# jpe17/TwoTowerMLRetrieval

Hardware: AMD Instinct MI355X
Metric: queries/sec top-k over 10M x 256-d docs (higher is better)
Workload: dtype f32 results (bit-identical to the fp32 FMA chain); f16-MFMA screen + fp32 rescoring; 1 GPU; exact cosine top-10 of B=1024 queries over 10000000 x 256 fp32 unit-norm passages resident in HBM (BASELINE configs[3]; configs[1] batch), row-sharded over 1 GPU(s), screened path (f16-MFMA filter + exact fp32 rescoring, bit-identical to the fp32 kernel); n_docs=10000000, dim=256, batch=1024, k=10, parallelism=rowshard1

## Files before the change

twotowermlretrieval_amd/csrc/score_topk.hip:

```cpp
#include "tt_common.h"

#include <limits.h>
#include <math.h>

namespace {

constexpr int TILE_DOCS = 32;
constexpr int SLAB_BYTES = 32 * 128;
constexpr int NSTAGE = 4;
#ifndef TT_K4_NT_NSTAGE
#define TT_K4_NT_NSTAGE 4
#endif
constexpr int NSTAGE_NT = TT_K4_NT_NSTAGE;
constexpr int WPB = 4;
constexpr int DMA_PER_SLAB = 4;
constexpr int PACE_R = 16;
constexpr int PACE_POLLS = 400;
constexpr int DRAW_POLLS = 1 << 16;
constexpr int DRAW_GAVE_UP = 0x7fffffff;

typedef __attribute__((address_space(3))) void lds_void;
typedef const __attribute__((address_space(1))) void gbl_void;

struct Cand;
// ... 723 lines not shown
            const int m = base + tid + u * MERGE_THREADS;
            ci[u] = m < end ? ix_at(m) : -1;
        }
#pragma unroll
        for (int u = 0; u < MERGE_SEG / MERGE_THREADS; ++u) {
            if (ci[u] >= 0) {
                const int slot = atomicAdd(&pool_n, 1);
                pool_v[slot] = v_at(base + tid + u * MERGE_THREADS);
                pool_i[slot] = ci[u];
            }
        }
        __syncthreads();
    }
    const int kept = reduce_pool();
    if (tid < k) {
        out_val[(size_t)b * k + tid] = tid < kept ? pool_v[tid] : -INFINITY;
        out_idx[(size_t)b * k + tid] = tid < kept ? pool_i[tid] : -1;
    }
}

__device__ __forceinline__ unsigned order_key(float f)
{
    const unsigned b = __float_as_uint(f);
    return (b & 0x80000000u) ? ~b : (b | 0x80000000u);
}

__device__ __forceinline__ float order_key_to_float(unsigned key)
{
    return __uint_as_float((key & 0x80000000u) ? (key & 0x7fffffffu) : ~key);
}

__global__ __launch_bounds__(256) void kth_largest_kernel(const float *__restrict__ vals, int M, int k,
                                                          float *__restrict__ out, const int *run_if,
                                                          float *__restrict__ top_out)
{
    if (run_if && run_if[blockIdx.x >> 5] == 0)
        return;
    __shared__ int hist[256];
    __shared__ int sel[2];
    __shared__ int wpos;
    const int row = blockIdx.x, tid = threadIdx.x, lane = tid & 63;
    const float *v = vals + (size_t)row * M;
    if (M < k) {
        if (tid == 0 && out)
            out[row] = -INFINITY;
        if (top_out)
            for (int i = tid; i < k; i += 256)
                top_out[(size_t)row * k + i] = i < M ? v[i] : -INFINITY;
        return;
    }
    unsigned prefix = 0u, mask = 0u;
    int k_rem = k;
    constexpr int KTH_REG = 16;
    const bool in_regs = M <= 256 * KTH_REG;
    unsigned keys[KTH_REG];
    if (in_regs) {
#pragma unroll
        for (int i = 0; i < KTH_REG; ++i) {
            const int m = tid + 256 * i;
            keys[i] = m < M ? order_key(v[m]) : 0u;
        }
    }
#pragma unroll 1
    for (int pass = 0; pass < 4; ++pass) {
        const int shift = 24 - 8 * pass;
        hist[tid] = 0;
        __syncthreads();
        if (in_regs) {
#pragma unroll
            for (int i = 0; i < KTH_REG; ++i)
                if (tid + 256 * i < M && (keys[i] & mask) == prefix)
                    atomicAdd(&hist[(keys[i] >> shift) & 255u], 1);
        } else {
            for (int m = tid; m < M; m += 256) {
                const unsigned key = order_key(v[m]);
                if ((key & mask) == prefix)
                    atomicAdd(&hist[(key >> shift) & 255u], 1);
            }
// ... 2 lines not shown
        if (tid < 64) {
            int c[4], s = 0;
#pragma unroll
            for (int i = 0; i < 4; ++i) {
                c[i] = hist[255 - (lane * 4 + i)];
                s += c[i];
            }
            int incl = s;
#pragma unroll
            for (int off = 1; off < 64; off <<= 1) {
                const int y = __shfl_up(incl, off);
                if (lane >= off)
                    incl += y;
            }
            int above = incl - s;
#pragma unroll
            for (int i = 0; i < 4; ++i) {
                if (above < k_rem && above + c[i] >= k_rem) {
                    sel[0] = 255 - (lane * 4 + i);
                    sel[1] = above;
                }
                above += c[i];
            }
        }
        __syncthreads();
        prefix |= (unsigned)sel[0] << shift;
        mask |= 0xffu << shift;
        k_rem -= sel[1];
        __syncthreads();
    }
    const float kth = order_key_to_float(prefix);
    if (tid == 0 && out)
        out[row] = kth;
    if (top_out) {
        if (tid == 0)
            wpos = 0;
        __syncthreads();
        float *dst = top_out + (size_t)row * k;
        if (in_regs) {
#pragma unroll
            for (int i = 0; i < KTH_REG; ++i)
                if (tid + 256 * i < M && keys[i] > prefix)
                    dst[atomicAdd(&wpos, 1)] = order_key_to_float(keys[i]);
        } else {
            for (int m = tid; m < M; m += 256)
                if (order_key(v[m]) > prefix)
                    dst[atomicAdd(&wpos, 1)] = v[m];
        }
        for (int i = k - k_rem + tid; i < k; i += 256)
            dst[i] = kth;
    }
}

__global__ __launch_bounds__(256) void score_rank_kernel(const float *__restrict__ Q,
                                                         const float *__restrict__ D, int N, int d,
                                                         const int64_t *__restrict__ target,
                                                         int64_t *rank)
{
    __shared__ float qs[512];
    __shared__ float stage[4][64 * 33];
    __shared__ int cnt[4];
    const int b = blockIdx.x, lane = threadIdx.x & 63, wv = threadIdx.x >> 6;
    const int tg = (int)target[b];
    for (int x = threadIdx.x; x < d; x += 256)
        qs[x] = Q[(size_t)b * d + x];
    __syncthreads();
// ... 471 lines not shown

int tt_score_topk_f32_pred(const float *Q, int B, int d, const float *D, int64_t N, int k, int64_t idx_offset,
                           float *out_val, int64_t *out_idx, void *workspace, size_t workspace_bytes,
                           const int *run_if, hipStream_t st)
{
    return score_topk_pred(Q, B, d, D, false, N, k, idx_offset, out_val, out_idx, workspace, workspace_bytes, run_if, st,
                           "tt_score_topk_f32");
}

int tt_score_topk_bf16_pred(const float *Q, int B, int d, const void *D, int64_t N, int k, int64_t idx_offset,
                            float *out_val, int64_t *out_idx, void *workspace, size_t workspace_bytes,
                            const int *run_if, hipStream_t st)
{
    return score_topk_pred(Q, B, d, D, true, N, k, idx_offset, out_val, out_idx, workspace, workspace_bytes, run_if, st,
                           "tt_score_topk_bf16");
}

TT_EXPORT int tt_score_topk_f32(const float *Q, int B, int d, const float *D, int64_t N, int k,
                                int64_t idx_offset, float *out_val, int64_t *out_idx, void *workspace,
                                size_t workspace_bytes, tt_stream_t stream)
{
    return tt_score_topk_f32_pred(Q, B, d, D, N, k, idx_offset, out_val, out_idx, workspace, workspace_bytes, nullptr,
                                  (hipStream_t)stream);
}

TT_EXPORT int tt_score_topk_bf16(const float *Q, int B, int d, const void *D_bf16, int64_t N, int k,
                                 int64_t idx_offset, float *out_val, int64_t *out_idx, void *workspace,
                                 size_t workspace_bytes, tt_stream_t stream)
{
    return tt_score_topk_bf16_pred(Q, B, d, D_bf16, N, k, idx_offset, out_val, out_idx, workspace, workspace_bytes,
                                   nullptr, (hipStream_t)stream);
}

int tt_kth_largest(const float *vals, int B, int M, int k, float *out, hipStream_t st)
{
    hipLaunchKernelGGL(kth_largest_kernel, dim3(B), dim3(256), 0, st, vals, M, k, out, (const int *)nullptr, (float *)nullptr);
    TT_LAUNCH_CHECK();
    return TT_OK;
}

int tt_k_largest_list(const float *vals, int B, int M, int k, float *list, hipStream_t st)
{
    hipLaunchKernelGGL(kth_largest_kernel, dim3(B), dim3(256), 0, st, vals, M, k, (float *)nullptr, (const int *)nullptr, list);
    TT_LAUNCH_CHECK();
    return TT_OK;
}

namespace {
__global__ __launch_bounds__(64) void seed_union_kernel(const float *__restrict__ lists, int world, int B, int ks, int kth,
                                                        float *__restrict__ seed)
{
    const int q = blockIdx.x, lane = threadIdx.x;
    const int M = world * ks;
    __shared__ float v[512];
    for (int i = lane; i < M; i += 64)
        v[i] = lists[((size_t)(i / ks) * B + q) * ks + (i % ks)];
    __syncthreads();
    for (int i = lane; i < M; i += 64) {
        const float x = v[i];
        int before = 0;
        for (int j = 0; j < M; ++j)
            before += (v[j] > x) || (v[j] == x && j < i);
        if (before == kth - 1)
            seed[q] = x;
    }
}
}

TT_EXPORT int tt_seed_union_f32(const float *lists, int world, int B, int list_len, int kth, float *seed, tt_stream_t stream)
// ... 754 lines not shown
```

twotowermlretrieval_amd/csrc/screen.hip:

```cpp
#include "tt_common.h"
#include <cmath>

#include <hip/hip_fp16.h>
#include <limits.h>
#include <math.h>

int tt_score_topk_f32_pred(const float *Q, int B, int d, const float *D, int64_t N, int k, int64_t idx_offset,
                           float *out_val, int64_t *out_idx, void *workspace, size_t workspace_bytes,
                           const int *run_if, hipStream_t st);
int tt_score_topk_bf16_pred(const float *Q, int B, int d, const void *D, int64_t N, int k, int64_t idx_offset,
                            float *out_val, int64_t *out_idx, void *workspace, size_t workspace_bytes,
                            const int *run_if, hipStream_t st);

int tt_kth_largest(const float *vals, int B, int M, int k, float *out, hipStream_t st);
int tt_k_largest_list(const float *vals, int B, int M, int k, float *list, hipStream_t st);

namespace {

typedef _Float16 h8 __attribute__((ext_vector_type(8)));
typedef _Float16 h4 __attribute__((ext_vector_type(4)));
typedef unsigned u32x4 __attribute__((ext_vector_type(4)));
typedef __attribute__((address_space(3))) void lds_void;
typedef const __attribute__((address_space(1))) void gbl_void;

#ifndef TT_SCREEN_STAGGER
#define TT_SCREEN_STAGGER 1
#endif
constexpr int SW = 8;
constexpr int STILE_BYTES = 32 * 512;
constexpr int SRING = 8;
constexpr int STPB = 2;
constexpr int SCAP = 128;
constexpr int SURV_MAX = 1024;
constexpr int POOL_MAX = 8192;
constexpr int FIN_MAX_CHUNKS = 2048;

struct SCand {
    float v;
    int x;
};

__device__ __forceinline__ float screen_eps(float qnorm, float dmax)
{
    return 1.10e-3f * qnorm * dmax + 1e-6f * (qnorm + dmax);
}

template <int NCH>
__device__ __forceinline__ void bf16_to_f16_lds(char *base, int lane)
{
    uint4 v[NCH];
#pragma unroll
    for (int i = 0; i < NCH; ++i)
        v[i] = *(const uint4 *)(base + (i * 64 + lane) * 16);
#pragma unroll
    for (int i = 0; i < NCH; ++i) {
        unsigned w[4] = {v[i].x, v[i].y, v[i].z, v[i].w};
#pragma unroll
        for (int e = 0; e < 4; ++e) {
            const _Float16 lo = (_Float16)__uint_as_float(w[e] << 16);
            const _Float16 hi = (_Float16)__uint_as_float(w[e] & 0xffff0000u);
            w[e] = (unsigned)__builtin_bit_cast(unsigned short, lo) | ((unsigned)__builtin_bit_cast(unsigned short, hi) << 16);
        }
        *(uint4 *)(base + (i * 64 + lane) * 16) = uint4{w[0], w[1], w[2], w[3]};
    }
}

__device__ __forceinline__ SCand scand_load_l2(const SCand *p)
{
    unsigned long long u = __hip_atomic_load((const unsigned long long *)p, __ATOMIC_RELAXED, __HIP_MEMORY_SCOPE_AGENT);
    SCand c;
    c.v = __uint_as_float((unsigned)u);
    c.x = (int)(u >> 32);
    return c;
}

struct ScreenParams {
    const float *Q;
    const _Float16 *D16;
    int B, N, k;
    int n_chunks, tiles_per_chunk, n_tiles;
    int static_tiles, tail_g, tail_blocks;
    int *tail_ctr;
    float dmax;
    SCand *cand;
    int *pcnt;
    int *flag;
    float *max_val;
    const float *thr0;
    int thr0_stride;
    const h8 *qimg;
    const float *qnorm;
    const float *dbg_thr;
};

__device__ __forceinline__ void scand_store_async(const SCand *base, unsigned byte_off, float v, int x)
{
    const unsigned long long bits = ((unsigned long long)(unsigned)x << 32) | (unsigned long long)__float_as_uint(v);
    asm volatile("global_store_dwordx2 %0, %1, %2\n\ts_nop 1" ::"v"(byte_off), "v"(bits), "s"(base) : "memory");
}

__device__ __forceinline__ void f32_store_async(float *dst, float v)
{
    asm volatile("global_store_dword %0, %1, off\n\ts_nop 0" ::"v"(dst), "v"(v) : "memory");
}

constexpr int SQUART = SCAP / 4;
constexpr int SQ_TRIGGER = SQUART - 10;
constexpr int SQ_KEEP_MAX = 4 * SQ_TRIGGER - 4;

__device__ __forceinline__ void screen_compact(SCand *base, const int (&n)[4], int k, float slack, int lane, int &n_new,
                                               float &thr_new, bool &have, bool &overflow)
{
    float v[2];
    int x[2], rank[2];
    bool live[2];
#pragma unroll
    for (int i = 0; i < 2; ++i) {
        v[i] = -INFINITY;
        x[i] = INT_MAX;
        rank[i] = 0;
        live[i] = (lane & 31) < ((lane >> 5) ? n[2 * i + 1] : n[2 * i]);
        if (live[i]) {
            const SCand c = scand_load_l2(base + 64 * i + lane);
            v[i] = c.v;
            x[i] = c.x;
        }
// ... 17 lines not shown
    overflow = false;
    n_new = total;
    thr_new = -INFINITY;
    if (have) {
        float kth = -INFINITY;
#pragma unroll
        for (int i = 0; i < 2; ++i) {
            const unsigned long long bk = __ballot(live[i] && rank[i] == k - 1);
            if (bk)
                kth = __builtin_bit_cast(float, __builtin_amdgcn_readlane(__builtin_bit_cast(int, v[i]), __ffsll((long long)bk) - 1));
        }
        thr_new = kth - slack;
        n_new = 0;
#pragma unroll
        for (int i = 0; i < 2; ++i)
            n_new += __popcll(__ballot(live[i] && v[i] >= thr_new));
        if (n_new > SQ_KEEP_MAX) {
            overflow = true;
            n_new = k;
        }
    }
#pragma unroll
    for (int i = 0; i < 2; ++i)
        if (live[i] && rank[i] < n_new) {
            SCand c;
            c.v = v[i];
            c.x = x[i];
            base[SQUART * (rank[i] & 3) + (rank[i] >> 2)] = c;
        }
}

__global__ __launch_bounds__(128) void q_image_kernel(const float *__restrict__ Q, int B, h8 *__restrict__ img,
                                                      float *__restrict__ qnorm, int *__restrict__ flag, int n_flags,
                                                      int *__restrict__ tail_ctr, int n_ctr)
{
    __shared__ int any_bad[2];
    if (blockIdx.x == 0)
        for (int i = threadIdx.x; i < n_ctr; i += 128)
            tail_ctr[i] = 0;
    const int lane = threadIdx.x & 63, wv = threadIdx.x >> 6;
    const int S = blockIdx.x * 2 + wv;
    const int g = lane >> 4, n = lane & 15;
    const int qrow = 16 * S + n;
    const bool live = qrow < B;
    const float *qp = Q + (size_t)min(qrow, B - 1) * 256 + 8 * g;
    float ss = 0.0f;
    bool bad = false;
#pragma unroll
    for (int s = 0; s < 8; ++s) {
        const f32x4 a = *(const f32x4 *)(qp + 32 * s);
        const f32x4 b = *(const f32x4 *)(qp + 32 * s + 4);
        h8 hv;
#pragma unroll
        for (int e = 0; e < 4; ++e) {
            const float x0 = live ? a[e] : 0.0f, x1 = live ? b[e] : 0.0f;
            ss += x0 * x0 + x1 * x1;
            bad |= !(fabsf(x0) <= 60000.0f) || !(fabsf(x1) <= 60000.0f);
            hv[e] = (_Float16)x0;
            hv[4 + e] = (_Float16)x1;
        }
        img[((size_t)S * 8 + s) * 64 + lane] = hv;
    }
    ss += __shfl_xor(ss, 16);
    ss += __shfl_xor(ss, 32);
    if (g == 0)
        qnorm[qrow] = sqrtf(ss);
    const bool wave_bad = __ballot(bad && live) != 0ull;
    if (lane == 0)
        any_bad[wv] = wave_bad ? 1 : 0;
    __syncthreads();
    if (threadIdx.x == 0 && (int)blockIdx.x < n_flags)
        flag[blockIdx.x] = (any_bad[0] | any_bad[1]) ? 2 : 0;
}

template <bool MAXONLY, int NSET, bool BF = false>
__global__ __launch_bounds__(SW * 64, 2) void screen_kernel(ScreenParams p)
{
    extern __shared__ __attribute__((aligned(16))) char ring[];
    constexpr int DMA_AUX = NSET < 3 ? 2 : 0;
    const int lane = threadIdx.x & 63;
    const int w = __builtin_amdgcn_readfirstlane(threadIdx.x >> 6);
    const int chunk = blockIdx.x % p.n_chunks;
    const int qgroup = blockIdx.x / p.n_chunks;
    int t0 = chunk * p.tiles_per_chunk;
    int t1 = min(t0 + p.tiles_per_chunk, p.static_tiles);
    __shared__ int next_block;
    const int k = p.k;
    const int g = lane >> 4, n = lane & 15;
    constexpr int QW = 16 * NSET, QB = SW * QW;
    const int qbase = qgroup * QB + w * QW;
    const bool wave_live = qbase < p.B;

    h8 qreg[NSET][8];
    float eps2[NSET];
    f32x4 negthr[NSET];
    int cnt[NSET];
#pragma unroll
    for (int c = 0; c < NSET; ++c)
        cnt[c] = 0;
#pragma unroll
    for (int c = 0; c < NSET; ++c) {
        const int qrow = qbase + 16 * c + n;
        const bool live = qrow < p.B;
        float qn = 0.0f;
        if (wave_live) {
            const h8 *src = p.qimg + ((size_t)(qbase / 16 + c) * 8) * 64 + lane;
#pragma unroll
            for (int s = 0; s < 8; ++s)
                qreg[c][s] = src[s * 64];
            qn = p.qnorm[qrow];
        }
        eps2[c] = 2.0f * screen_eps(qn, p.dmax);
        const float floor_thr = -(1.01f * qn * p.dmax + 1e-30f);
        const float t_init = live ? ((!MAXONLY && p.thr0) ? fmaxf(p.thr0[(size_t)qrow * p.thr0_stride + p.thr0_stride - 1] - eps2[c], floor_thr)
                                                    : floor_thr)
                            : INFINITY;
        float c_init = -t_init;
        if (MAXONLY)
            c_init = (p.dbg_thr && live) ? -p.dbg_thr[qrow] : 0.0f;
        negthr[c] = f32x4{c_init, c_init, c_init, c_init};
    }

    SCand *const cwave = p.cand + ((size_t)blockIdx.x * QB + w * QW) * SCAP;

    auto compact_where = [&](int c, unsigned qmask) {
        asm volatile("s_waitcnt vmcnt(0)" ::: "memory");
        while (qmask) {
            const int q = __ffs((int)qmask) - 1;
            qmask &= qmask - 1;
            const int nq[4] = {__builtin_amdgcn_readlane(cnt[c], q), __builtin_amdgcn_readlane(cnt[c], q + 16),
                               __builtin_amdgcn_readlane(cnt[c], q + 32), __builtin_amdgcn_readlane(cnt[c], q + 48)};
            const float slack = __builtin_bit_cast(float, __builtin_amdgcn_readlane(__builtin_bit_cast(int, eps2[c]), q));
            int n_new;
            float tn;
            bool have, ovf;
            screen_compact(cwave + (size_t)(16 * c + q) * SCAP, nq, k, slack, lane, n_new, tn, have, ovf);
            if (ovf && lane == 0)
                atomicOr(p.flag + ((qbase + 16 * c) >> 5), 1);
            if (n == q) {
                cnt[c] = (n_new - g + 3) >> 2;
                if (have)
                    negthr[c] = f32x4{-tn, -tn, -tn, -tn};
            }
        }
    };

    const char *D = (const char *)p.D16;
    const char *rowp[2];
    auto set_rows = [&](int tile) {
#pragma unroll
        for (int i = 0; i < 2; ++i) {
            const int row = 2 * (2 * w + i) + (lane >> 5);
            const int doc = min(tile * 32 + row, p.N - 1);
            const int chunk16 = (lane & 31) ^ (row & 15);
            rowp[i] = D + (size_t)doc * 512 + chunk16 * 16;
        }
    };
    auto dma_issue = [&](int tile, int stage) {
        set_rows(min(tile, t1 - 1));
        char *dst = ring + stage * STILE_BYTES + (2 * w) * 1024;
        __builtin_amdgcn_global_load_lds((gbl_void *)rowp[0], (lds_void *)dst, 16, 0, DMA_AUX);
        __builtin_amdgcn_global_load_lds((gbl_void *)rowp[1], (lds_void *)(dst + 1024), 16, 0, DMA_AUX);
    };
    auto dma_piece = [&](int i, int stage) {
        char *dst = ring + stage * STILE_BYTES + (2 * w + i) * 1024;
        __builtin_amdgcn_global_load_lds((gbl_void *)rowp[i], (lds_void *)dst, 16, 0, DMA_AUX);
    };

    for (;;) {
    if (t0 < t1) {
#pragma unroll
        for (int gi = 0; gi < SRING - STPB; ++gi)
            dma_issue(t0 + gi, gi);
        int stage = 0;
        const int rd_base = n * 512;
        f32x4 acc[2][NSET];
        const bool late = TT_SCREEN_STAGGER && w >= 4;
        bool pending = false;
        int ptile = 0;
        auto epilogue = [&](int tile) {
                const int tile_base = tile * 32;
            const bool partial = tile_base + 32 > p.N;
            if (!MAXONLY) {
                if (partial) {
#pragma unroll
                    for (int u = 0; u < 2; ++u)
#pragma unroll
                        for (int r = 0; r < 4; ++r)
                            if (tile_base + 16 * u + 4 * g + r >= p.N) {
#pragma unroll
                                for (int c = 0; c < NSET; ++c)
                                    acc[u][c][r] = -INFINITY;
                            }
                }
                int mall = INT_MIN;
#pragma unroll
                for (int u = 0; u < 2; ++u)
#pragma unroll
                    for (int c = 0; c < NSET; ++c)
#pragma unroll
                        for (int r = 0; r < 4; ++r)
                            mall = max(mall, __float_as_int(acc[u][c][r]));
                if (__ballot(mall >= 0) != 0ull) {
#pragma unroll
                    for (int c = 0; c < NSET; ++c) {
                        int mu[2];
#pragma unroll
                        for (int u = 0; u < 2; ++u)
                            mu[u] = max(max(__float_as_int(acc[u][c][0]), __float_as_int(acc[u][c][1])),
                                        max(__float_as_int(acc[u][c][2]), __float_as_int(acc[u][c][3])));
                        if (__ballot(max(mu[0], mu[1]) >= 0) == 0ull)
                            continue;
                        const unsigned mine = (unsigned)(((16 * c + n) * SCAP + SQUART * g) * sizeof(SCand));
                        const float thr_c = -negthr[c][0];
#pragma unroll
                        for (int u = 0; u < 2; ++u) {
                            if (__ballot(mu[u] >= 0) == 0ull)
                                continue;
#pragma unroll
                            for (int r = 0; r < 4; ++r) {
                                if (__float_as_int(acc[u][c][r]) >= 0) {
                                    scand_store_async(cwave, mine + (unsigned)cnt[c] * (unsigned)sizeof(SCand),
                                                      acc[u][c][r] + thr_c, tile_base + 16 * u + 4 * g + r);
                                    ++cnt[c];
                                }
                            }
                        }
                        unsigned long long full = __ballot(cnt[c] > SQ_TRIGGER);
                        full = (full | (full >> 32));
                        full = (full | (full >> 16)) & 0xffffull;
                        if (full)
                            compact_where(c, (unsigned)full);
                    }
                }
            } else {
#pragma unroll
                for (int c = 0; c < NSET; ++c) {
                    float m = -INFINITY;
                    if (!partial) {
                        int mi = INT_MIN;
#pragma unroll
                        for (int u = 0; u < 2; ++u)
#pragma unroll
                            for (int r = 0; r < 4; ++r)
                                mi = max(mi, __float_as_int(acc[u][c][r]));
                        m = __int_as_float(mi);
                    } else {
#pragma unroll
                        for (int u = 0; u < 2; ++u)
#pragma unroll
                            for (int r = 0; r < 4; ++r)
                                m = fmaxf(m, tile_base + 16 * u + 4 * g + r < p.N ? acc[u][c][r] : -INFINITY);
                    }
                    m = fmaxf(m, __shfl_xor(m, 16));
                    m = fmaxf(m, __shfl_xor(m, 32));
                    const int qrow = qbase + 16 * c + n;
                    if (g == 0 && qrow < p.B)
                        f32_store_async(p.max_val + (size_t)qrow * p.n_tiles + tile, m);
                }
            }
                };
        for (int tile = t0; tile < t1; ++tile) {
            if ((tile - t0) % STPB == 0) {
                asm volatile("s_waitcnt vmcnt(%0)" ::"n"(2 * (SRING - 2 * STPB)) : "memory");
                if (BF && tile == t0) {
#pragma unroll
                    for (int i = 0; i < STPB; ++i)
                        bf16_to_f16_lds<2>(ring + ((stage + i) % SRING) * STILE_BYTES + (2 * w) * 1024, lane);
                    asm volatile("s_waitcnt lgkmcnt(0)" ::: "memory");
                }
                __builtin_amdgcn_s_barrier();
            } else if (BF && (tile - t0) % STPB == STPB - 1) {
                asm volatile("s_waitcnt vmcnt(%0)" ::"n"(2 * (SRING - 3 * STPB + 1)) : "memory");
#pragma unroll
                for (int i = 1; i <= STPB; ++i)
                    bf16_to_f16_lds<2>(ring + ((stage + i) % SRING) * STILE_BYTES + (2 * w) * 1024, lane);
                asm volatile("s_waitcnt lgkmcnt(0)" ::: "memory");
            }
            const int fill_stage = (stage + SRING - STPB) % SRING;
            set_rows(min(tile + SRING - STPB, t1 - 1));
            if (!wave_live) {
                dma_piece(0, fill_stage);
                dma_piece(1, fill_stage);
            }
            if (wave_live) {
                if (late && pending)
                    epilogue(ptile);
                const char *buf = ring + stage * STILE_BYTES + rd_base;
                h8 a0[3], a1[3];
                auto a_read = [&](int s) {
                    const int off = ((4 * s + g) ^ n) << 4;
                    a0[s % 3] = *(const h8 *)(buf + off);
                    a1[s % 3] = *(const h8 *)(buf + 16 * 512 + off);
                };
                a_read(0);
                a_read(1);
#pragma unroll
                for (int s = 0; s < 8; ++s) {
                    if (s + 2 < 8)
                        a_read(s + 2);
                    if (s == 2)
                        dma_piece(0, fill_stage);
                    if (s == 6)
                        dma_piece(1, fill_stage);
                    __builtin_amdgcn_sched_barrier(0);
#pragma unroll
                    for (int c = 0; c < NSET; ++c) {
                        const f32x4 c0 = s == 0 ? negthr[c] : acc[0][c];
                        const f32x4 c1 = s == 0 ? negthr[c] : acc[1][c];
                        acc[0][c] = __builtin_amdgcn_mfma_f32_16x16x32_f16(a0[s % 3], qreg[c][s], c0, 0, 0, 0);
                        acc[1][c] = __builtin_amdgcn_mfma_f32_16x16x32_f16(a1[s % 3], qreg[c][s], c1, 0, 0, 0);
                    }
                    __builtin_amdgcn_sched_barrier(0);
                }
                if (late) {
                    pending = true;
                    ptile = tile;
                } else {
                    epilogue(tile);
                }
            }
            stage = (stage + 1) % SRING;
        }
        if (wave_live && late && pending)
            epilogue(ptile);
    }
    if (MAXONLY || p.tail_blocks == 0)
        break;
    asm volatile("s_waitcnt vmcnt(0)" ::: "memory");
    __builtin_amdgcn_s_barrier();
    if (threadIdx.x == 0)
        next_block = atomicAdd(p.tail_ctr + qgroup, 1);
    __syncthreads();
    const int blk = next_block;
    if (blk >= p.tail_blocks)
        break;
    t0 = p.static_tiles + blk * p.tail_g;
    t1 = min(t0 + p.tail_g, p.n_tiles);
    }
    asm volatile("s_waitcnt vmcnt(0)" ::: "memory");
    __builtin_amdgcn_s_barrier();

    if (MAXONLY)
        return;
#pragma unroll
    for (int c = 0; c < NSET; ++c) {
        int tot = cnt[c] + __shfl_xor(cnt[c], 16);
        tot += __shfl_xor(tot, 32);
        const unsigned long long over = __ballot(tot > k) & 0xffffull;
        if (over)
            compact_where(c, (unsigned)over);
        int packed = cnt[c] << (8 * g);
        packed |= __shfl_xor(packed, 16);
        packed |= __shfl_xor(packed, 32);
        const int qrow = qbase + 16 * c + n;
        if (g == 0 && qrow < p.B)
            p.pcnt[(size_t)qrow * p.n_chunks + chunk] = packed;
    }
}

constexpr int TW = 4;
constexpr int TSLAB_BYTES = 32 * 128;
constexpr int TSTAGE = 4;
constexpr int TDMA = 4;
constexpr int TSTREAM_AUX = 2;

template <bool MAXONLY, int NQS = 2, bool BF = false>
__global__ __launch_bounds__(TW * 64, 2) void screen_stream_kernel(ScreenParams p)
{
    constexpr int QPT = 16 * NQS;
    extern __shared__ __attribute__((aligned(16))) char ring_all[];
    const int lane = threadIdx.x & 63;
    const int w = __builtin_amdgcn_readfirstlane(threadIdx.x >> 6);
    char *const ring = ring_all + w * (TSTAGE * TSLAB_BYTES);
    const int task = blockIdx.x * TW + w;
    const int n_qtiles = (p.B + QPT - 1) / QPT;
    if (task >= n_qtiles * p.n_chunks)
        return;
    const int qtile = task / p.n_chunks, chunk = task % p.n_chunks;
    const int t0 = chunk * p.tiles_per_chunk;
    const int t1 = min(t0 + p.tiles_per_chunk, p.n_tiles);
    const int k = p.k;
    const int g = lane >> 4, n = lane & 15;
    const int qbase = qtile * QPT;

    h8 qreg[NQS][8];
    float eps2[NQS];
    f32x4 negthr[NQS];
// ... 503 lines not shown
            if (out16)
                *(h4 *)(out16 + row * d + x) = hv;
        }
#pragma unroll
        for (int off = 32; off >= 1; off >>= 1)
            ss += __shfl_xor(ss, off);
        nmax = fmaxf(nmax, sqrtf(ss));
    }
#pragma unroll
    for (int off = 32; off >= 1; off >>= 1)
        amax = fmaxf(amax, __shfl_xor(amax, off));
    if (lane == 0) {
        red[wave] = nmax;
        red[4 + wave] = amax;
    }
    __syncthreads();
    if (threadIdx.x == 0 && stats) {
        atomicMax(stats, __float_as_uint(fmaxf(fmaxf(red[0], red[1]), fmaxf(red[2], red[3]))));
        atomicMax(stats + 1, __float_as_uint(fmaxf(fmaxf(red[4], red[5]), fmaxf(red[6], red[7]))));
    }
}

struct SPlan {
    bool stream;
    int nset;
    int n_qgroups;
    int q_per_block;
    int n_tiles, n_chunks, tiles_per_chunk;
    int static_tiles, tail_g, tail_blocks;
    size_t tailctr_off;
    bool sample;
    int s_tiles, s_chunks, s_tiles_per_chunk;
    int64_t s_docs;
    size_t cand_off, pcnt_off, smax_val_off, sthr_val_off, qimg_off, qnorm_off, stats_off, ws_bytes;
    int rows_pad;
};

constexpr int64_t SAMPLE_MIN_N = 65536;
constexpr int STREAM_MAX_B = 64;

int one_round(bool stream, int n_qgroups)
{
    return stream ? (tt_device_cus() * 2 * TW + n_qgroups - 1) / n_qgroups : (tt_device_cus() + n_qgroups - 1) / n_qgroups;
}

SPlan make_splan(int B, int64_t N, int k)
{
    SPlan pl;
    pl.stream = B <= STREAM_MAX_B;
    if (B <= SW * 32) {
        pl.nset = B <= SW * 16 ? 1 : 2;
    } else {
        const int groups = (B + SW * 64 - 1) / (SW * 64);
        pl.nset = (B + groups - 1) / groups <= SW * 48 ? 3 : 4;
    }
    pl.q_per_block = pl.stream ? (B <= 32 ? 32 : 64) : SW * 16 * pl.nset;
    pl.n_qgroups = (B + pl.q_per_block - 1) / pl.q_per_block;
    pl.n_tiles = (int)((N + 31) / 32);
    int max_chunks = pl.stream && N >= SAMPLE_MIN_N ? FIN_MAX_CHUNKS : POOL_MAX / (k + 16);
    if (!pl.stream)
        max_chunks = max_chunks > 255 ? 255 : max_chunks;
    const TTChunks c = tt_chunks(pl.n_tiles, one_round(pl.stream, pl.n_qgroups), max_chunks);
    pl.n_chunks = c.n_chunks;
    const TTTailSplit t = tt_tail_split(c.tiles_per_chunk, c.n_chunks, pl.n_tiles,
                                        pl.stream ? 0 : TT_AB_SWITCH(TT_SCREEN_TAIL_DIV, 8), 16, 8, 32);
    pl.tiles_per_chunk = t.own;
    pl.static_tiles = t.static_tiles;
    pl.tail_g = t.tail_g;
    pl.tail_blocks = t.tail_blocks;
    const int n_tasks = pl.n_qgroups * pl.n_chunks;
    const size_t rows = (size_t)pl.n_qgroups * pl.q_per_block;
    pl.rows_pad = (int)rows;
    pl.sample = N >= SAMPLE_MIN_N;
    int64_t s_docs = N / 64;
    const int per_k = k <= 16 ? 4096 : 2048;
    const int64_t s_min = (int64_t)k * per_k < N / 4 ? (int64_t)k * per_k : N / 4;
    s_docs = s_docs < s_min ? s_min : s_docs;
    s_docs = s_docs < 32 ? 32 : s_docs;
    pl.s_docs = (s_docs + 31) / 32 * 32;
    pl.s_tiles = (int)(pl.s_docs / 32);
    const TTChunks sc = tt_chunks(pl.s_tiles, one_round(pl.stream, pl.n_qgroups), INT_MAX);
    pl.s_tiles_per_chunk = sc.tiles_per_chunk;
    pl.s_chunks = pl.sample ? sc.n_chunks : 0;
    TTWorkspace ws;
    pl.cand_off = ws.take((size_t)n_tasks * pl.q_per_block * SCAP * sizeof(SCand));
    pl.pcnt_off = ws.take(rows * pl.n_chunks * sizeof(int));
    pl.smax_val_off = ws.take(rows * (size_t)(pl.sample ? pl.s_tiles : 1) * sizeof(float));
    pl.sthr_val_off = ws.take(rows * sizeof(float));
    pl.qimg_off = ws.take(rows * 256 * sizeof(_Float16));
    pl.qnorm_off = ws.take(rows * sizeof(float));
    pl.tailctr_off = ws.take((size_t)pl.n_qgroups * sizeof(int));
    pl.stats_off = ws.take(rows * 2 * sizeof(int));
    pl.ws_bytes = ws.off;
    return pl;
}

template <bool MAXONLY, bool BF>
const void *screen_fn(bool stream, int q_per_block, int nset)
{
    if (stream)
        return q_per_block == 64 ? (const void *)screen_stream_kernel<MAXONLY, 4, BF>
                                 : (const void *)screen_stream_kernel<MAXONLY, 2, BF>;
    switch (nset) {
    case 4: return (const void *)screen_kernel<MAXONLY, 4, BF>;
    case 3: return (const void *)screen_kernel<MAXONLY, 3, BF>;
    case 2: return (const void *)screen_kernel<MAXONLY, 2, BF>;
    default: return (const void *)screen_kernel<MAXONLY, 1, BF>;
    }
}

int launch_screen(bool stream, int q_per_block, int nset, bool maxonly, ScreenParams p, int n_tasks, hipStream_t st,
                  bool bf16 = false)
{
    const void *fn = maxonly ? (bf16 ? screen_fn<true, true>(stream, q_per_block, nset) : screen_fn<true, false>(stream, q_per_block, nset))
                             : (bf16 ? screen_fn<false, true>(stream, q_per_block, nset) : screen_fn<false, false>(stream, q_per_block, nset));
    const size_t lds = stream ? (size_t)TW * TSTAGE * TSLAB_BYTES : (size_t)SRING * STILE_BYTES;
    const int blocks = stream ? (n_tasks + TW - 1) / TW : n_tasks;
    TT_HIP_CHECK(hipFuncSetAttribute(fn, hipFuncAttributeMaxDynamicSharedMemorySize, (int)lds));
    void *args[] = {&p};
    TT_HIP_CHECK(hipLaunchKernel(fn, dim3(blocks), dim3((stream ? TW : SW) * 64), args, lds, st));
    return TT_OK;
}

}

// ... 85 lines not shown
    if (seed_only && (k_seed < 1 || k_seed > k))
        return tt_fail(TT_ERR_BAD_SHAPE, "%s: k_seed=%d outside [1, k=%d]", who, k_seed, k);
    const SPlan pl = make_splan(B, N, k);
    const size_t need = pl.ws_bytes + (bf16 ? tt_score_topk_bf16_workspace_bytes(B, N, d, k) : tt_score_topk_workspace_bytes(B, N, d, k));
    if (!workspace || workspace_bytes < need || ((uintptr_t)workspace & 255) || (bf16 && ((uintptr_t)D16 & 15)))
        return tt_fail(TT_ERR_WORKSPACE, "%s: workspace %zu < %zu bytes", who, workspace_bytes, need);
    char *ws = (char *)workspace;
    const int k_thr = phase == Phase::SeedThreshold ? k_seed : k;
    float *thr_out = phase == Phase::SeedThreshold ? seed : (float *)(ws + pl.sthr_val_off);

    ScreenParams sp;
    sp.Q = Q;
    sp.D16 = (const _Float16 *)D16;
    sp.B = B;
    sp.N = (int)N;
    sp.k = k;
    sp.n_chunks = pl.n_chunks;
    sp.tiles_per_chunk = pl.tiles_per_chunk;
    sp.n_tiles = pl.n_tiles;
    sp.static_tiles = pl.static_tiles;
    sp.tail_g = pl.tail_g;
    sp.tail_blocks = pl.tail_blocks;
    sp.tail_ctr = (int *)(ws + pl.tailctr_off);
    sp.dmax = dmax_norm;
    sp.cand = (SCand *)(ws + pl.cand_off);
    sp.pcnt = (int *)(ws + pl.pcnt_off);
    sp.flag = fallback_flag;
    sp.max_val = nullptr;
    sp.thr0 = nullptr;
    sp.thr0_stride = k;
    sp.qimg = (const h8 *)(ws + pl.qimg_off);
    sp.qnorm = (const float *)(ws + pl.qnorm_off);
    sp.dbg_thr = nullptr;
    if (caller_seed) {
        sp.thr0 = seed;
        sp.thr0_stride = 1;
    } else {
        hipLaunchKernelGGL(q_image_kernel, dim3(pl.rows_pad / 32), dim3(128), 0, st, Q, B, (h8 *)(ws + pl.qimg_off),
                           (float *)(ws + pl.qnorm_off), fallback_flag, (B + 31) / 32, (int *)(ws + pl.tailctr_off),
                           pl.n_qgroups);
        TT_LAUNCH_CHECK();
        if (pl.sample) {
            ScreenParams ss = sp;
            ss.N = (int)pl.s_docs;
            ss.n_tiles = pl.s_tiles;
            ss.n_chunks = pl.s_chunks;
            ss.tiles_per_chunk = pl.s_tiles_per_chunk;
            ss.static_tiles = pl.s_tiles;
            ss.tail_blocks = 0;
            ss.max_val = (float *)(ws + pl.smax_val_off);
            TT_RC_CHECK(launch_screen(pl.stream, pl.q_per_block, pl.nset, true, ss, pl.n_qgroups * pl.s_chunks, st, bf16));
            if (phase == Phase::SeedList)
                TT_RC_CHECK(tt_k_largest_list(ss.max_val, B, pl.s_tiles, k_seed, seed, st));
            else
                TT_RC_CHECK(tt_kth_largest(ss.max_val, B, pl.s_tiles, k_thr, thr_out, st));
            sp.thr0 = (const float *)(ws + pl.sthr_val_off);
            sp.thr0_stride = 1;
        } else if (seed_only) {
            const int n = phase == Phase::SeedList ? B * k_seed : B;
            hipLaunchKernelGGL(seed_fill_kernel, dim3((n + 255) / 256), dim3(256), 0, st, seed, n);
            TT_LAUNCH_CHECK();
        }
    }
    if (seed_only)
        return TT_OK;
    if (prof_events)
        TT_HIP_CHECK(hipEventRecord((hipEvent_t)prof_events[0], st));
    TT_RC_CHECK(launch_screen(pl.stream, pl.q_per_block, pl.nset, false, sp, pl.n_qgroups * pl.n_chunks, st, bf16));
    if (prof_events)
        TT_HIP_CHECK(hipEventRecord((hipEvent_t)prof_events[1], st));

    FinishParams fp;
    fp.Q = Q;
    fp.D32 = bf16 ? nullptr : (const float *)D32;
    fp.Dbf = bf16 ? (const unsigned *)D32 : nullptr;
    fp.B = B;
    fp.N = (int)N;
    fp.k = k;
    fp.n_chunks = pl.n_chunks;
    fp.q_per_block = pl.q_per_block;
    fp.dmax = dmax_norm;
    fp.cand = sp.cand;
    fp.pcnt = sp.pcnt;
    fp.flag = fallback_flag;
    fp.idx_offset = idx_offset;
    fp.out_val = out_val;
    fp.out_idx = out_idx;
    fp.stats = (int *)(ws + pl.stats_off);
    hipLaunchKernelGGL(screen_finish_kernel, dim3(B), dim3(256), (size_t)(2 * pl.n_chunks + 1) * sizeof(int), st, fp);
    TT_LAUNCH_CHECK();
// ... 132 lines not shown
{
    hipStream_t st = (hipStream_t)stream;
    DbgPlan pl;
    if (B <= 0 || N <= 0 || N >= (int64_t)INT_MAX - 64 || !make_dbg_plan(B, N, form, pl))
        return tt_fail(TT_ERR_BAD_SHAPE, "tt_debug_screen_s16: B=%d N=%lld form=%d", B, (long long)N, form);
    if (!Q || !D16 || !out_t)
        return tt_fail(TT_ERR_BAD_SHAPE, "tt_debug_screen_s16: null pointer");
    if (!workspace || workspace_bytes < pl.total || ((uintptr_t)workspace & 255))
        return tt_fail(TT_ERR_WORKSPACE, "tt_debug_screen_s16: workspace %zu < %zu bytes", workspace_bytes, pl.total);
    char *ws = (char *)workspace;
    ScreenParams sp;
    sp.Q = Q;
    sp.D16 = (const _Float16 *)D16;
    sp.B = B;
    sp.N = (int)N;
    sp.k = 1;
    sp.n_chunks = pl.n_chunks;
    sp.tiles_per_chunk = pl.tiles_per_chunk;
    sp.n_tiles = pl.n_tiles;
    sp.static_tiles = pl.n_tiles;
    sp.tail_g = 1;
    sp.tail_blocks = 0;
    sp.tail_ctr = nullptr;
    sp.dmax = dmax_norm;
    sp.cand = nullptr;
    sp.pcnt = nullptr;
    sp.flag = (int *)(ws + pl.flag_off);
    sp.max_val = out_t;
    sp.thr0 = nullptr;
    sp.thr0_stride = 1;
    sp.qimg = (const h8 *)(ws + pl.qimg_off);
    sp.qnorm = (const float *)(ws + pl.qnorm_off);
    sp.dbg_thr = thr;
    hipLaunchKernelGGL(q_image_kernel, dim3(pl.rows_pad / 32), dim3(128), 0, st, Q, B, (h8 *)(ws + pl.qimg_off),
                       (float *)(ws + pl.qnorm_off), sp.flag, pl.rows_pad / 32, (int *)nullptr, 0);
    TT_LAUNCH_CHECK();
    return launch_screen(form == 0, pl.q_per_block, form, true, sp, pl.n_qgroups * pl.n_chunks, st, bf16);
}
}

TT_EXPORT int tt_debug_screen_s16(const float *Q, int B, const void *D16, int64_t N, float dmax_norm, const float *thr,
                                  int form, float *out_t, void *workspace, size_t workspace_bytes, tt_stream_t stream)
{
    return debug_screen(Q, B, D16, N, dmax_norm, thr, form, out_t, workspace, workspace_bytes, stream, false);
}

TT_EXPORT int tt_debug_screen_s16_bf16(const float *Q, int B, const void *D_bf16, int64_t N, float dmax_norm, const float *thr,
                                       int form, float *out_t, void *workspace, size_t workspace_bytes, tt_stream_t stream)
{
    return debug_screen(Q, B, D_bf16, N, dmax_norm, thr, form, out_t, workspace, workspace_bytes, stream, true);
}
```

Measured before the change: 262,800 queries/s.

## Tighten screen threshold online via per-query global score histograms

Adds a per-query 16-bin global histogram of screened candidate scores, built from atomic adds issued in the screen epilogue. Every 64 tiles each wave reads the histogram and raises its per-query threshold to the lowest bin edge that holds at least k hits. The bin width comes from a new spread output of the kth-largest kernel run on the sample pass. The aim is to cut survivors and compaction work sooner than local compaction alone would, at the cost of extra global atomics and polling. It also staggers the in-loop DMA issue slots per wave.

```diff
diff --git a/twotowermlretrieval_amd/csrc/score_topk.hip b/twotowermlretrieval_amd/csrc/score_topk.hip
--- a/twotowermlretrieval_amd/csrc/score_topk.hip
+++ b/twotowermlretrieval_amd/csrc/score_topk.hip
@@ -779,18 +779,22 @@
 
 __global__ __launch_bounds__(256) void kth_largest_kernel(const float *__restrict__ vals, int M, int k,
                                                           float *__restrict__ out, const int *run_if,
-                                                          float *__restrict__ top_out)
+                                                          float *__restrict__ top_out,
+                                                          float *__restrict__ spread_out = nullptr)
 {
     if (run_if && run_if[blockIdx.x >> 5] == 0)
         return;
     __shared__ int hist[256];
     __shared__ int sel[2];
     __shared__ int wpos;
+    __shared__ unsigned top_key;
     const int row = blockIdx.x, tid = threadIdx.x, lane = tid & 63;
     const float *v = vals + (size_t)row * M;
     if (M < k) {
         if (tid == 0 && out)
             out[row] = -INFINITY;
+        if (tid == 0 && spread_out)
+            spread_out[row] = 0.0f;
         if (top_out)
             for (int i = tid; i < k; i += 256)
                 top_out[(size_t)row * k + i] = i < M ? v[i] : -INFINITY;
@@ -859,6 +863,26 @@
     const float kth = order_key_to_float(prefix);
     if (tid == 0 && out)
         out[row] = kth;
+    if (spread_out) {
+        if (tid == 0)
+            top_key = 0u;
+        __syncthreads();
+        unsigned mk = 0u;
+        if (in_regs) {
+#pragma unroll
+            for (int i = 0; i < KTH_REG; ++i)
+                mk = max(mk, keys[i]);
+        } else {
+            for (int m = tid; m < M; m += 256)
+                mk = max(mk, order_key(v[m]));
+        }
+        atomicMax(&top_key, mk);
+        __syncthreads();
+        if (tid == 0) {
+            const float sp = (order_key_to_float(top_key) - kth) * 0.125f;
+            spread_out[row] = sp >= 0.0f && sp < 3.0e38f ? sp : 0.0f;
+        }
+    }
     if (top_out) {
         if (tid == 0)
             wpos = 0;
@@ -1396,9 +1420,10 @@
                                    nullptr, (hipStream_t)stream);
 }
 
-int tt_kth_largest(const float *vals, int B, int M, int k, float *out, hipStream_t st)
-{
-    hipLaunchKernelGGL(kth_largest_kernel, dim3(B), dim3(256), 0, st, vals, M, k, out, (const int *)nullptr, (float *)nullptr);
+int tt_kth_largest(const float *vals, int B, int M, int k, float *out, float *spread_out, hipStream_t st)
+{
+    hipLaunchKernelGGL(kth_largest_kernel, dim3(B), dim3(256), 0, st, vals, M, k, out, (const int *)nullptr, (float *)nullptr,
+                       spread_out);
     TT_LAUNCH_CHECK();
     return TT_OK;
 }
diff --git a/twotowermlretrieval_amd/csrc/screen.hip b/twotowermlretrieval_amd/csrc/screen.hip
--- a/twotowermlretrieval_amd/csrc/screen.hip
+++ b/twotowermlretrieval_amd/csrc/screen.hip
@@ -12,7 +12,7 @@
                             float *out_val, int64_t *out_idx, void *workspace, size_t workspace_bytes,
                             const int *run_if, hipStream_t st);
 
-int tt_kth_largest(const float *vals, int B, int M, int k, float *out, hipStream_t st);
+int tt_kth_largest(const float *vals, int B, int M, int k, float *out, float *spread_out, hipStream_t st);
 int tt_k_largest_list(const float *vals, int B, int M, int k, float *list, hipStream_t st);
 
 namespace {
@@ -34,6 +34,8 @@
 constexpr int SURV_MAX = 1024;
 constexpr int POOL_MAX = 8192;
 constexpr int FIN_MAX_CHUNKS = 2048;
+constexpr int SHIST_BINS = 16;
+constexpr int SHIST_R = 64;
 
 struct SCand {
     float v;
@@ -91,7 +93,25 @@
     const h8 *qimg;
     const float *qnorm;
     const float *dbg_thr;
+    int *hist;
+    const float *hist_w;
+    int hist_r;
+    int dma_slots;
 };
+
+#ifdef TT_AB
+#define TT_SCREEN_HIST_R_OF(p) ((p).hist_r)
+#define TT_SCREEN_DMA_SLOTS_OF(p) ((p).dma_slots)
+#else
+#define TT_SCREEN_HIST_R_OF(p) SHIST_R
+#define TT_SCREEN_DMA_SLOTS_OF(p) 1
+#endif
+
+__device__ __forceinline__ void hist_add_async(const int *base, unsigned byte_off)
+{
+    int one;
+    asm volatile("v_mov_b32 %0, 1\n\tglobal_atomic_add %1, %0, %2\n\ts_nop 0" : "=&v"(one) : "v"(byte_off), "s"(base) : "memory");
+}
 
 __device__ __forceinline__ void scand_store_async(const SCand *base, unsigned byte_off, float v, int x)
 {
@@ -175,12 +195,15 @@
 
 __global__ __launch_bounds__(128) void q_image_kernel(const float *__restrict__ Q, int B, h8 *__restrict__ img,
                                                       float *__restrict__ qnorm, int *__restrict__ flag, int n_flags,
-                                                      int *__restrict__ tail_ctr, int n_ctr)
+                                                      int *__restrict__ tail_ctr, int n_ctr, int *__restrict__ hist)
 {
     __shared__ int any_bad[2];
     if (blockIdx.x == 0)
         for (int i = threadIdx.x; i < n_ctr; i += 128)
             tail_ctr[i] = 0;
+    if (hist)
+        for (int i = threadIdx.x; i < 32 * SHIST_BINS; i += 128)
+            hist[(size_t)blockIdx.x * 32 * SHIST_BINS + i] = 0;
     const int lane = threadIdx.x & 63, wv = threadIdx.x >> 6;
     const int S = blockIdx.x * 2 + wv;
     const int g = lane >> 4, n = lane & 15;
@@ -235,7 +258,7 @@
     const bool wave_live = qbase < p.B;
 
     h8 qreg[NSET][8];
-    float eps2[NSET];
+    float eps2 = 0.0f;
     f32x4 negthr[NSET];
     int cnt[NSET];
 #pragma unroll
@@ -253,9 +276,11 @@
                 qreg[c][s] = src[s * 64];
             qn = p.qnorm[qrow];
         }
-        eps2[c] = 2.0f * screen_eps(qn, p.dmax);
+        const float eps2_c = 2.0f * screen_eps(qn, p.dmax);
+        if ((lane >> 4) == c)
+            eps2 = eps2_c;
         const float floor_thr = -(1.01f * qn * p.dmax + 1e-30f);
-        const float t_init = live ? ((!MAXONLY && p.thr0) ? fmaxf(p.thr0[(size_t)qrow * p.thr0_stride + p.thr0_stride - 1] - eps2[c], floor_thr)
+        const float t_init = live ? ((!MAXONLY && p.thr0) ? fmaxf(p.thr0[(size_t)qrow * p.thr0_stride + p.thr0_stride - 1] - eps2_c, floor_thr)
                                                     : floor_thr)
                             : INFINITY;
         float c_init = -t_init;
@@ -265,6 +290,49 @@
     }
 
     SCand *const cwave = p.cand + ((size_t)blockIdx.x * QB + w * QW) * SCAP;
+
+    const int hist_r = TT_SCREEN_HIST_R_OF(p);
+    const bool hist_on = !MAXONLY && hist_r > 0 && p.hist && p.thr0;
+    __shared__ float2 hist_bins[MAXONLY ? 1 : QB];
+    float2 *const hbw = hist_bins + (MAXONLY ? 0 : w * QW);
+    if (hist_on && wave_live && lane < QW) {
+        const int ql = qbase + lane;
+        hbw[lane] = float2{p.thr0[(size_t)min(ql, p.B - 1) * p.thr0_stride + p.thr0_stride - 1],
+                           fmaxf(p.hist_w ? p.hist_w[ql] : 0.0f, eps2)};
+    }
+    const int *const hwave = p.hist + (hist_on ? (size_t)qbase * SHIST_BINS : 0);
+    auto hist_refresh = [&]() {
+        float x = -INFINITY;
+        int ln = lane;
+        asm volatile("" : "+v"(ln));
+        if (ln < QW && qbase + ln < p.B) {
+            const unsigned long long *hp = (const unsigned long long *)(hwave + ln * SHIST_BINS);
+            int cum = 0, best = -1;
+#pragma unroll
+            for (int h = 1; h >= 0; --h) {
+                unsigned long long u[SHIST_BINS / 4];
+#pragma unroll
+                for (int j = 0; j < SHIST_BINS / 4; ++j)
+                    u[j] = __hip_atomic_load(hp + h * (SHIST_BINS / 4) + j, __ATOMIC_RELAXED, __HIP_MEMORY_SCOPE_AGENT);
+#pragma unroll
+                for (int b = SHIST_BINS / 2 - 1; b >= 0; --b) {
+                    cum += (int)(u[b >> 1] >> (32 * (b & 1)));
+                    if (cum >= k && best < 0)
+                        best = h * (SHIST_BINS / 2) + b;
+                }
+                asm volatile("" : "+v"(cum), "+v"(best)::"memory");
+            }
+            const float2 lw = hbw[ln];
+            if (best >= 0)
+                x = fmaf((float)best, lw.y, lw.x) - eps2;
+        }
+#pragma unroll
+        for (int c = 0; c < NSET; ++c) {
+            const float tn = __shfl(x, 16 * c + n);
+            if (-tn < negthr[c][0])
+                negthr[c] = f32x4{-tn, -tn, -tn, -tn};
+        }
+    };
 
     auto compact_where = [&](int c, unsigned qmask) {
         asm volatile("s_waitcnt vmcnt(0)" ::: "memory");
@@ -273,7 +341,7 @@
             qmask &= qmask - 1;
             const int nq[4] = {__builtin_amdgcn_readlane(cnt[c], q), __builtin_amdgcn_readlane(cnt[c], q + 16),
                                __builtin_amdgcn_readlane(cnt[c], q + 32), __builtin_amdgcn_readlane(cnt[c], q + 48)};
-            const float slack = __builtin_bit_cast(float, __builtin_amdgcn_readlane(__builtin_bit_cast(int, eps2[c]), q));
+            const float slack = __builtin_bit_cast(float, __builtin_amdgcn_readlane(__builtin_bit_cast(int, eps2), 16 * c + q));
             int n_new;
             float tn;
             bool have, ovf;
@@ -282,7 +350,7 @@
                 atomicOr(p.flag + ((qbase + 16 * c) >> 5), 1);
             if (n == q) {
                 cnt[c] = (n_new - g + 3) >> 2;
-                if (have)
+                if (have && (!hist_on || -tn < negthr[c][0]))
                     negthr[c] = f32x4{-tn, -tn, -tn, -tn};
             }
         }
@@ -310,6 +378,10 @@
         __builtin_amdgcn_global_load_lds((gbl_void *)rowp[i], (lds_void *)dst, 16, 0, DMA_AUX);
     };
 
+    const int dma_slot = TT_SCREEN_DMA_SLOTS_OF(p) == 1 ? (w < 4 ? w : ((w + 2) & 3))
+                         : TT_SCREEN_DMA_SLOTS_OF(p) == 2 ? (w < 4 ? 2 : 0)
+                                                          : 2;
+    bool pool_block = false;
     for (;;) {
     if (t0 < t1) {
 #pragma unroll
@@ -321,6 +393,7 @@
         const bool late = TT_SCREEN_STAGGER && w >= 4;
         bool pending = false;
         int ptile = 0;
+        int hist_due = pool_block ? 0 : hist_r;
         auto epilogue = [&](int tile) {
                 const int tile_base = tile * 32;
             const bool partial = tile_base + 32 > p.N;
@@ -356,6 +429,14 @@
                             continue;
                         const unsigned mine = (unsigned)(((16 * c + n) * SCAP + SQUART * g) * sizeof(SCand));
                         const float thr_c = -negthr[c][0];
+                        float lo_c = 0.0f, w_c = 0.0f;
+                        int nn = n;
+                        if (hist_on) {
+                            asm volatile("" : "+v"(nn));
+                            const float2 lw = hbw[16 * c + nn];
+                            lo_c = lw.x;
+                            w_c = lw.y;
+                        }
 #pragma unroll
                         for (int u = 0; u < 2; ++u) {
                             if (__ballot(mu[u] >= 0) == 0ull)
@@ -363,9 +444,16 @@
 #pragma unroll
                             for (int r = 0; r < 4; ++r) {
                                 if (__float_as_int(acc[u][c][r]) >= 0) {
-                                    scand_store_async(cwave, mine + (unsigned)cnt[c] * (unsigned)sizeof(SCand),
-                                                      acc[u][c][r] + thr_c, tile_base + 16 * u + 4 * g + r);
+                                    const float sc = acc[u][c][r] + thr_c;
+                                    scand_store_async(cwave, mine + (unsigned)cnt[c] * (unsigned)sizeof(SCand), sc,
+                                                      tile_base + 16 * u + 4 * g + r);
                                     ++cnt[c];
+                                    if (hist_on && sc >= lo_c) {
+                                        int b = (int)fminf((sc - lo_c) * __builtin_amdgcn_rcpf(w_c), (float)(SHIST_BINS - 1));
+                                        b = max(b - (sc >= fmaf((float)b, w_c, lo_c) ? 0 : 1), 0);
+                                        if (sc >= fmaf((float)b, w_c, lo_c))
+                                            hist_add_async(hwave + 16 * c * SHIST_BINS, (unsigned)((nn * SHIST_BINS + b) * sizeof(int)));
+                                    }
                                 }
                             }
                         }
@@ -429,6 +517,13 @@
             if (wave_live) {
                 if (late && pending)
                     epilogue(ptile);
+                if (hist_on) {
+                    if (hist_due == 0) {
+                        hist_refresh();
+                        hist_due = hist_r;
+                    }
+                    --hist_due;
+                }
                 const char *buf = ring + stage * STILE_BYTES + rd_base;
                 h8 a0[3], a1[3];
                 auto a_read = [&](int s) {
@@ -438,13 +533,15 @@
                 };
                 a_read(0);
                 a_read(1);
+                int slot = dma_slot;
+                asm volatile("" : "+s"(slot));
 #pragma unroll
                 for (int s = 0; s < 8; ++s) {
                     if (s + 2 < 8)
                         a_read(s + 2);
-                    if (s == 2)
+                    if (s == slot)
                         dma_piece(0, fill_stage);
-                    if (s == 6)
+                    if (s == slot + 4)
                         dma_piece(1, fill_stage);
                     __builtin_amdgcn_sched_barrier(0);
 #pragma unroll
@@ -478,6 +575,7 @@
     const int blk = next_block;
     if (blk >= p.tail_blocks)
         break;
+    pool_block = true;
     t0 = p.static_tiles + blk * p.tail_g;
     t1 = min(t0 + p.tail_g, p.n_tiles);
     }
@@ -496,7 +594,9 @@
         int packed = cnt[c] << (8 * g);
         packed |= __shfl_xor(packed, 16);
         packed |= __shfl_xor(packed, 32);
-        const int qrow = qbase + 16 * c + n;
+        int nf = lane & 15;
+        asm volatile("" : "+v"(nf));
+        const int qrow = qbase + 16 * c + nf;
         if (g == 0 && qrow < p.B)
             p.pcnt[(size_t)qrow * p.n_chunks + chunk] = packed;
     }
@@ -1066,7 +1166,7 @@
     bool sample;
     int s_tiles, s_chunks, s_tiles_per_chunk;
     int64_t s_docs;
-    size_t cand_off, pcnt_off, smax_val_off, sthr_val_off, qimg_off, qnorm_off, stats_off, ws_bytes;
+    size_t cand_off, pcnt_off, smax_val_off, sthr_val_off, qimg_off, qnorm_off, stats_off, hist_off, histw_off, ws_bytes;
     int rows_pad;
 };
 
@@ -1125,6 +1225,8 @@
     pl.qnorm_off = ws.take(rows * sizeof(float));
     pl.tailctr_off = ws.take((size_t)pl.n_qgroups * sizeof(int));
     pl.stats_off = ws.take(rows * 2 * sizeof(int));
+    pl.hist_off = ws.take(rows * SHIST_BINS * sizeof(int));
+    pl.histw_off = ws.take(rows * sizeof(float));
     pl.ws_bytes = ws.off;
     return pl;
 }
@@ -1276,13 +1378,17 @@
     sp.qimg = (const h8 *)(ws + pl.qimg_off);
     sp.qnorm = (const float *)(ws + pl.qnorm_off);
     sp.dbg_thr = nullptr;
+    sp.hist = pl.stream ? nullptr : (int *)(ws + pl.hist_off);
+    sp.hist_w = nullptr;
+    sp.hist_r = TT_AB_SWITCH(TT_SCREEN_HIST_R, SHIST_R);
+    sp.dma_slots = TT_AB_SWITCH(TT_SCREEN_DMA_SLOTS, 1);
     if (caller_seed) {
         sp.thr0 = seed;
         sp.thr0_stride = 1;
     } else {
         hipLaunchKernelGGL(q_image_kernel, dim3(pl.rows_pad / 32), dim3(128), 0, st, Q, B, (h8 *)(ws + pl.qimg_off),
                            (float *)(ws + pl.qnorm_off), fallback_flag, (B + 31) / 32, (int *)(ws + pl.tailctr_off),
-                           pl.n_qgroups);
+                           pl.n_qgroups, sp.hist);
         TT_LAUNCH_CHECK();
         if (pl.sample) {
             ScreenParams ss = sp;
@@ -1297,9 +1403,11 @@
             if (phase == Phase::SeedList)
                 TT_RC_CHECK(tt_k_largest_list(ss.max_val, B, pl.s_tiles, k_seed, seed, st));
             else
-                TT_RC_CHECK(tt_kth_largest(ss.max_val, B, pl.s_tiles, k_thr, thr_out, st));
+                TT_RC_CHECK(tt_kth_largest(ss.max_val, B, pl.s_tiles, k_thr, thr_out,
+                                           phase == Phase::Whole ? (float *)(ws + pl.histw_off) : nullptr, st));
             sp.thr0 = (const float *)(ws + pl.sthr_val_off);
             sp.thr0_stride = 1;
+            sp.hist_w = (const float *)(ws + pl.histw_off);
         } else if (seed_only) {
             const int n = phase == Phase::SeedList ? B * k_seed : B;
             hipLaunchKernelGGL(seed_fill_kernel, dim3((n + 255) / 256), dim3(256), 0, st, seed, n);
@@ -1498,8 +1606,12 @@
     sp.qimg = (const h8 *)(ws + pl.qimg_off);
     sp.qnorm = (const float *)(ws + pl.qnorm_off);
     sp.dbg_thr = thr;
+    sp.hist = nullptr;
+    sp.hist_w = nullptr;
+    sp.hist_r = 0;
+    sp.dma_slots = TT_AB_SWITCH(TT_SCREEN_DMA_SLOTS, 1);
     hipLaunchKernelGGL(q_image_kernel, dim3(pl.rows_pad / 32), dim3(128), 0, st, Q, B, (h8 *)(ws + pl.qimg_off),
-                       (float *)(ws + pl.qnorm_off), sp.flag, pl.rows_pad / 32, (int *)nullptr, 0);
+                       (float *)(ws + pl.qnorm_off), sp.flag, pl.rows_pad / 32, (int *)nullptr, 0, (int *)nullptr);
     TT_LAUNCH_CHECK();
     return launch_screen(form == 0, pl.q_per_block, form, true, sp, pl.n_qgroups * pl.n_chunks, st, bf16);
 }
```

Result: slower. 255,700 queries/s (-2.7%).
